# RedhawkSDR/psk_soft

Hardware: AMD Instinct MI355X
Metric: complex IQ Msamples/s, QPSK 8 sps, 4096 ch; % HBM roofline at 1/2/4/8 GPUs (higher is better)
Workload: dtype f32

## Files before the change

### psk_soft_amd/csrc/psk_capi.cpp

```cpp
#include <hip/hip_runtime_api.h>
#include <hip/hip_vector_types.h>

#include <atomic>
#include <cmath>
#include <condition_variable>
#include <cstdio>
#include <cstdlib>
#include <cstring>
#include <functional>
#include <mutex>
#include <new>
#include <string>
#include <thread>
#include <vector>

#include "psk_acquire.h"
#include "psk_symrate.h"
#include "psk_ctl.h"
#include "psk_gather.h"
#include "psk_plan.h"
#include "psk_quality.h"
#include "psk_soft_hip.h"
#include "psk_fir.h"
#include "psk_resample.h"
// ... 18 lines not shown
                             float2 *t_s, PfChan *pf_chan, uint32_t tile0, hipStream_t stream);
hipError_t launch_tile_front_any(const ChanPlan *plans, const uint32_t *list, uint32_t ch0, uint32_t nch, uint32_t max_tiles, uint32_t max_S,
                                 const ChanState *states, const float2 *rings, uint32_t ring_cap, TileInfo *tiles, float *t_raw, float2 *t_s,
                                 PfChan *pf_chan, hipStream_t stream);
hipError_t launch_tile_fit(const ChanPlan *plans, const uint32_t *list, uint32_t ch0, uint32_t nch, ChanState *states, float2 *rings,
                           uint32_t ring_cap, float *yvs, uint32_t fit_cap, uint32_t y_len, TileInfo *tiles, const float *t_raw,
                           const float2 *t_s, float *t_est, const PfScratch &sc, hipStream_t stream);
hipError_t launch_wide_front(const ChanPlan *plans, const uint32_t *list, uint32_t ch0, uint32_t nch, uint32_t max_tiles, uint32_t max_S,
                             const float2 *rings, uint32_t ring_cap, TileInfo *tiles, float *t_raw, float2 *t_s, PfChan *pf_chan, void *rec,
                             void *wst, hipStream_t stream);
size_t wide_rec_bytes();
size_t wide_stat_bytes();
uint32_t wide_chunks(uint32_t S);
hipError_t launch_seq_wide(const void *plans, const uint32_t *list, uint32_t ch0, uint32_t nch, void *states, float2 *rings,
                           uint32_t ring_cap, float *yvs, uint32_t fit_cap, double *symE, uint32_t symE_stride, hipStream_t stream);
hipError_t launch_pfit(const ChanPlan *plans, const uint32_t *list, uint32_t ch0, uint32_t nch, uint32_t max_tiles, ChanState *states,
                       float2 *rings, uint32_t ring_cap, float *yvs, uint32_t fit_cap, uint32_t y_len, TileInfo *tiles, const float *t_raw,
                       const float2 *t_s, float *t_est, const PfScratch &sc, bool second_round, hipStream_t stream);
hipError_t launch_tile_fit_range(const ChanPlan *plans, const uint32_t *list, uint32_t ch0, uint32_t nch, ChanState *states, float2 *rings,
                                 uint32_t ring_cap, float *yvs, uint32_t fit_cap, uint32_t y_len, TileInfo *tiles, const float *t_raw,
                                 const float2 *t_s, float *t_est, void *carry, float *carry_y, uint32_t tile0, uint32_t ntiles,
                                 hipStream_t stream);
size_t pipe_carry_bytes();
hipError_t launch_far_fit(const ChanPlan *plans, const uint32_t *list, uint32_t ch0, uint32_t nch, ChanState *states, float2 *rings,
                          uint32_t ring_cap, float *yvs, uint32_t fit_cap, float *far_y, uint32_t far_rows, TileInfo *tiles,
                          const float *t_raw, const float2 *t_s, float *t_est, hipStream_t stream);
hipError_t launch_far_quiet(const ChanPlan *plans, const uint32_t *list, uint32_t ch0, uint32_t nch, ChanState *states, float2 *rings,
                            uint32_t ring_cap, float *yvs, uint32_t fit_cap, float *far_y, uint32_t far_rows, hipStream_t stream);
size_t far_ring_bytes();
hipError_t launch_tile_back(const ChanPlan *plans, const uint32_t *list, uint32_t ch0, uint32_t nch, uint32_t max_tiles,
                            const ChanState *states, const TileInfo *tiles, const float2 *t_s, const float *t_est, uint32_t tile0,
                            uint32_t early, hipStream_t stream);
}
// ... 1024 lines not shown
    p.mode = p.S == 1u ? psk::PLAN_SEQ_S1 : psk::PLAN_SEQ;
    p.lf_flags &= ~(uint32_t)(psk::PLAN_TILED | psk::PLAN_PFIT | psk::PLAN_ANYFRONT | psk::PLAN_FARFIT);
}
psk_soft_status scratch_tiles(Round &r)
{
    psk_soft_handle *const h = r.h;
    PlanSummary &res = r.res;
    if (!r.tile_syms || (r.tile_syms <= h->tile_sym_cap && r.tile_count <= h->tile_cap && r.pf_syms <= h->pf_sym_cap && r.pf_count <= h->pf_cap))
        return PSK_SOFT_OK;
    h->tile_cap = h->tile_sym_cap = h->pf_cap = h->pf_sym_cap = 0;
    const size_t syms = plus_quarter(r.tile_syms), cnt = plus_quarter(r.tile_count);
    const size_t psyms = plus_quarter(r.pf_syms) + 128u, pcnt = plus_quarter(r.pf_count) + 1u;
    psk::PfScratch &pf = h->pf;
    bool got = false;
    PSK_HIP(grow_scratch({scratch_buf(&h->d_tiles, cnt), scratch_buf(&h->d_traw, syms), scratch_buf(&h->d_test, syms), scratch_buf(&h->d_ts, syms),
                          scratch_buf(&pf.k, psyms), scratch_buf(&pf.y, psyms), scratch_buf(&pf.S, psyms), scratch_buf(&pf.c, psyms),
                          scratch_buf(&pf.tt, psyms), scratch_buf(&pf.xs, psyms), scratch_buf(&pf.tile, pcnt),
                          scratch_buf(&pf.blk, psyms / 128u + 1u), scratch_buf(&pf.walk, psyms / 128u + 1u)},
                         &got));
    if (got && !pf.chan) {
        got = hipMalloc((void **)&pf.chan, sizeof(psk::PfChan) * h->nch) == hipSuccess &&
              hipMemset(pf.chan, 0, sizeof(psk::PfChan) * h->nch) == hipSuccess && hipHostMalloc((void **)&pf.hint, 64) == hipSuccess;
        if (got)
            *pf.hint = 0u;
    }
    if (got) {
        h->tile_cap = cnt, h->tile_sym_cap = syms, h->pf_cap = pcnt, h->pf_sym_cap = psyms;
        return PSK_SOFT_OK;
    }
    (void)hipGetLastError();
    for (uint32_t i = 0; i < r.nch; i++) {
        psk::ChanPlan &p = r.plans[i];
// ... 351 lines not shown
    psk_soft_handle *const h = r.h;
    const uint32_t *const l = r.d_list + s.off;
    const uint32_t ring_cap = h->lim.ring_cap, fit_cap = h->lim.fit_cap;
    PSK_HIP(mark(r, st, t.front, t.S, t.H, s.off, s.cnt, s.tiles_max, t.y_len, t.r_front));
    if (front == Front::window_class)
        PSK_HIP(psk::launch_tile_front(t.S, class_H(t.H), r.d_plans, l, r.ch0, s.cnt, s.tiles_max, h->d_state, h->d_ring, ring_cap, t.r_len, h->d_tiles,
                                       h->d_traw, h->d_ts, h->pf.chan, 0u, st));
    else if (front == Front::any)
        PSK_HIP(psk::launch_tile_front_any(r.d_plans, l, r.ch0, s.cnt, s.tiles_max, s.max_S, h->d_state, h->d_ring, ring_cap, h->d_tiles, h->d_traw,
                                           h->d_ts, h->pf.chan, st));
    else
        PSK_HIP(psk::launch_wide_front(r.d_plans, l, r.ch0, s.cnt, s.tiles_max, s.max_S, h->d_ring, ring_cap, h->d_tiles, h->d_traw, h->d_ts,
                                       h->pf.chan, h->d_wide_rec, h->d_wide_stat, st));
    if (fit == Fit::lds && h->opt_pfit) {
        PSK_HIP(mark(r, st, t.pfit, t.S, t.H, s.off, s.cnt, s.tiles_max, t.y_len, r.pf_second));
        PSK_HIP(psk::launch_pfit(r.d_plans, l, r.ch0, s.cnt, s.tiles_max, h->d_state, h->d_ring, ring_cap, h->d_yv, fit_cap, t.y_len, h->d_tiles,
                                 h->d_traw, h->d_ts, h->d_test, h->pf, r.pf_second, st));
    }
    PSK_HIP(mark(r, st, t.fit, t.S, t.H, s.off, s.cnt, s.tiles_max, t.y_len, t.r_len));
    if (fit == Fit::lds)
        PSK_HIP(psk::launch_tile_fit(r.d_plans, l, r.ch0, s.cnt, h->d_state, h->d_ring, ring_cap, h->d_yv, fit_cap, t.y_len, h->d_tiles, h->d_traw,
                                     h->d_ts, h->d_test, h->pf, st));
    else
        PSK_HIP(psk::launch_far_fit(r.d_plans, l, r.ch0, s.cnt, h->d_state, h->d_ring, ring_cap, h->d_yv, fit_cap, h->d_far_y, h->far_rows_cap,
                                    h->d_tiles, h->d_traw, h->d_ts, h->d_test, st));
    PSK_HIP(mark(r, st, t.back, t.S, t.H, s.off, s.cnt, s.tiles_max, t.y_len, t.r_len));
    PSK_HIP(psk::launch_tile_back(r.d_plans, l, r.ch0, s.cnt, s.tiles_max, h->d_state, h->d_tiles, h->d_ts, h->d_test, 0u, 0u, st));
    return PSK_SOFT_OK;
}
psk_soft_status enqueue_any_sets(const Round &r)
{
    psk_soft_handle *const h = r.h;
// ... 402 lines not shown
            if (h->ev_up[s]) (void)hipEventDestroy(h->ev_up[s]);
        }
        if (h->d_state) (void)hipFree(h->d_state);
        if (h->d_ring) (void)hipFree(h->d_ring);
        if (h->d_yv) (void)hipFree(h->d_yv);
        h->qpass.free();
        if (h->d_quality) (void)hipFree(h->d_quality);
        h->apass.free();
        if (h->d_acquire) (void)hipFree(h->d_acquire);
        h->spass.free();
        if (h->d_symrate) (void)hipFree(h->d_symrate);
        if (h->d_tiles) (void)hipFree(h->d_tiles);
        if (h->d_traw) (void)hipFree(h->d_traw);
        if (h->d_test) (void)hipFree(h->d_test);
        if (h->d_ts) (void)hipFree(h->d_ts);
        for (void *q : {(void *)h->pf.k, (void *)h->pf.y, (void *)h->pf.S, (void *)h->pf.c, (void *)h->pf.tt, (void *)h->pf.xs,
                        (void *)h->pf.tile, (void *)h->pf.blk, (void *)h->pf.walk, (void *)h->pf.chan})
            if (q) (void)hipFree(q);
        if (h->pf.hint) (void)hipHostFree(h->pf.hint);
        if (h->tile_ev) (void)hipEventDestroy(h->tile_ev);
        for (auto &cv : h->cvt) cv.free();
        for (auto &g : h->gat) g.free();
        for (auto &g : h->gdesc) g.free();
        if (h->d_tune_tab) (void)hipFree(h->d_tune_tab);
        h->rs_hist.free();
        if (h->d_fir_taps) (void)hipFree(h->d_fir_taps);
        h->fir_hist.free();
        for (auto &sl : h->stage) {
            if (sl.stream) (void)hipStreamSynchronize(sl.stream);
            if (sl.h_buf) (void)hipHostFree(sl.h_buf);
            if (sl.d_buf) (void)hipFree(sl.d_buf);
// ... 1959 lines not shown
```

### psk_soft_amd/csrc/psk_pfit.h

```cpp
#ifndef PSK_PFIT_H
#define PSK_PFIT_H

#include "psk_fast_kernel.h"

namespace psk {

constexpr uint32_t kPfFailYSum = 1u, kPfFailXySum = 2u, kPfFailUnwrap = 4u;

PSK_DEV bool pf_mine(const ChanPlan &p) { return p.mode == PLAN_FAST && (p.lf_flags & PLAN_PFIT) && p.n_out != 0; }
PSK_DEV bool pf_in_round(const ChanPlan &p, const PfScratch &sc, uint32_t bi, int round) { return pf_mine(p) && (round == 0 || sc.chan[bi].retry != 0u); }

struct PfGeo {
    int lane, n_out, n_blocks, c_begin, c_end, tile;
    uint64_t off;
    uint32_t tbase;
    uint32_t bbase;
};
PSK_DEV bool pf_geo(const ChanPlan &p, PfGeo &g)
{
    g.lane = threadIdx.x & 63;
    g.n_out = (int)p.n_out;
    g.n_blocks = (g.n_out + kB - 1) / kB;
    g.tile = (int)blockIdx.x;
    g.c_begin = g.tile * (int)p.tile_blocks;
    g.c_end = g.c_begin + (int)p.tile_blocks < g.n_blocks ? g.c_begin + (int)p.tile_blocks : g.n_blocks;
// ... 6 lines not shown
{
    const int n = (int)p.lf_n;
    return t >= n ? y_row[t - n] : yv[(p.lf_head + (uint32_t)t) % fit_cap];
}

constexpr float kPfSteep = 0.12f;
__global__ __launch_bounds__(64) void pf_unwrap_kernel(const ChanPlan *__restrict__ plans, const uint32_t *__restrict__ list, uint32_t ch0,
                                                       const ChanState *__restrict__ states, const float *__restrict__ t_raw, PfScratch sc)
{
    const uint32_t bi = list[blockIdx.y];
    const ChanPlan &p = plans[bi];
    PfGeo g;
    if (!pf_mine(p) || !pf_geo(p, g))
        return;
    const float *raw_row = t_raw + g.off;
    int *k_row = sc.k + g.off;
    const float inv2pi = 0.15915494f, two_pi = 6.2831853f;
    const ChanState &st = states[ch0 + bi];
    const bool steep = !(__builtin_fabsf(st.lf_m) < kPfSteep);
    int run = 0;
    if (steep) {
        for (int c = g.c_begin; c < g.c_end; c++) {
            const int i0 = c * kB + 2 * g.lane;
            const float2 rw = *reinterpret_cast<const float2 *>(raw_row + i0);
            const float before = c ? raw_row[c * kB - 1] : rw.x;
            const float prev = wave_up1(rw.y, before);
            int j0 = (int)__builtin_rintf((prev - rw.x) * inv2pi);
            const int j1 = (int)__builtin_rintf((rw.x - rw.y) * inv2pi);
            if (i0 == 0)
                j0 = 0;
            const int incl = wave_scan_i32(j0 + j1);
// ... 28 lines not shown
            const float U = a + two_pi * (float)(K - run);
            const float U_l = bperm_addr(((g.lane & ~7) - 8) << 2, U), U_r = bperm_addr(((g.lane & ~7) + 8) << 2, U);
            const float slope = grp == 0 ? (U_r - U) * (1.0f / 16.0f) : grp == 7 ? (U - U_l) * (1.0f / 16.0f) : (U_r - U_l) * (1.0f / 32.0f);
            const float dt0 = (float)(2 * (g.lane & 7)) - 7.5f;
            const float line0 = a + slope * dt0, line1 = line0 + slope;
            const int k0 = K + (int)__builtin_rintf((line0 - rw.x) * inv2pi), k1 = K + (int)__builtin_rintf((line1 - rw.y) * inv2pi);
            *reinterpret_cast<int2 *>(k_row + i0) = make_int2(k0, k1);
            run = __builtin_amdgcn_readlane(K, 63);
            a_last = read_lane(a, 63);
        }
    }
    if (g.lane == 0)
        sc.tile[g.tbase + g.tile].jsum = run;
}

__global__ __launch_bounds__(64) void pf_y_kernel(const ChanPlan *__restrict__ plans, const uint32_t *__restrict__ list, uint32_t ch0,
                                                  const ChanState *__restrict__ states, const float *__restrict__ t_raw, PfScratch sc, int round)
{
    const uint32_t bi = list[blockIdx.y];
    const ChanPlan &p = plans[bi];
    PfGeo g;
    if (!pf_in_round(p, sc, bi, round) || !pf_geo(p, g))
        return;
    const float *raw_row = t_raw + g.off;
    int *k_row = sc.k + g.off;
    float *y_row = sc.y + g.off;
    int koff = 0;
    if (round == 0) {
        for (int j = g.lane; j < g.tile; j += kWave) koff += sc.tile[g.tbase + j].jsum;
        koff = __builtin_amdgcn_readlane(wave_scan_i32(koff), 63);
        if (!(__builtin_fabsf(states[ch0 + bi].lf_m) < kPfSteep))
            koff += (int)unwrap_count(states[ch0 + bi].phaseEstimate, (double)raw_row[0]);
    }
    float2 rw_n = *reinterpret_cast<const float2 *>(raw_row + g.c_begin * kB + 2 * g.lane);
    int2 k_n = *reinterpret_cast<const int2 *>(k_row + g.c_begin * kB + 2 * g.lane);
    for (int c = g.c_begin; c < g.c_end; c++) {
        const int i0 = c * kB + 2 * g.lane;
        const float2 rw = rw_n;
        int2 k = k_n;
        if (c + 1 < g.c_end) {
            rw_n = *reinterpret_cast<const float2 *>(raw_row + i0 + kB);
            k_n = *reinterpret_cast<const int2 *>(k_row + i0 + kB);
        }
        k.x += koff;
        k.y += koff;
        *reinterpret_cast<int2 *>(k_row + i0) = k;
        const double two_pi = PSK_KD(kTwoPi, c);
        const float y0 = (float)((double)rw.x + (double)(long long)k.x * two_pi);
        const float y1 = (float)((double)rw.y + (double)(long long)k.y * two_pi);
        *reinterpret_cast<float2 *>(y_row + i0) = make_float2(y0, y1);
    }
}

__global__ __launch_bounds__(64) void pf_ydiff_kernel(const ChanPlan *__restrict__ plans, const uint32_t *__restrict__ list, uint32_t ch0,
                                                      const float *__restrict__ yvs, uint32_t fit_cap, PfScratch sc, int round)
{
    const uint32_t bi = list[blockIdx.y];
    const ChanPlan &p = plans[bi];
    PfGeo g;
    if (!pf_in_round(p, sc, bi, round) || !pf_geo(p, g))
        return;
    const float *y_row = sc.y + g.off;
    const float *yv = yvs + (size_t)(ch0 + bi) * fit_cap;
    double *S_row = sc.S + g.off;
    double run = 0.0, dlast = 0.0;
    const int j0 = g.c_begin * kB + 2 * g.lane;
    float2 y_n = *reinterpret_cast<const float2 *>(y_row + j0);
    float z0_n = pf_z(p, y_row, yv, fit_cap, j0), z1_n = pf_z(p, y_row, yv, fit_cap, j0 + 1);
    for (int c = g.c_begin; c < g.c_end; c++) {
        const int i0 = c * kB + 2 * g.lane;
        const float2 y = y_n;
        const float z0 = z0_n, z1 = z1_n;
        if (c + 1 < g.c_end) {
            y_n = *reinterpret_cast<const float2 *>(y_row + i0 + kB);
            z0_n = pf_z(p, y_row, yv, fit_cap, i0 + kB);
// ... 11 lines not shown
        dlast = read_lane((last & 1) ? a0 + d1 : a0, last >> 1);
    }
    if (g.lane == 0) {
        sc.tile[g.tbase + g.tile].dsum = run;
        sc.tile[g.tbase + g.tile].dlast = dlast;
    }
}

__global__ __launch_bounds__(64) void pf_ysum_kernel(const ChanPlan *__restrict__ plans, const uint32_t *__restrict__ list, uint32_t ch0,
                                                     const ChanState *__restrict__ states, const float *__restrict__ yvs, uint32_t fit_cap,
                                                     PfScratch sc, int round)
{
    const uint32_t bi = list[blockIdx.y];
    const ChanPlan &p = plans[bi];
    PfGeo g;
    if (!pf_in_round(p, sc, bi, round) || !pf_geo(p, g))
        return;
    const float *y_row = sc.y + g.off;
    const float *yv = yvs + (size_t)(ch0 + bi) * fit_cap;
    double *S_row = sc.S + g.off;
    double *c_row = sc.c + g.off;
    float *t_row = sc.tt + g.off;
    double soff = 0.0;
    for (int j = g.lane; j < g.tile; j += kWave) soff += sc.tile[g.tbase + j].dsum;
    soff = sc.chan[bi].ySum_c + wave_sum_f64(soff);
    bool bad = false;
    if (g.tile > 0) {
        double soff_b = 0.0;
        for (int j = g.lane; j < g.tile - 1; j += kWave) soff_b += sc.tile[g.tbase + j].dsum;
        soff_b = sc.chan[bi].ySum_c + wave_sum_f64(soff_b);
        bad = !same_bits(soff_b + sc.tile[g.tbase + g.tile - 1].dlast, soff);
    }
    const float xd = p.lf_xdelta;
    const float sizef = (float)(p.lf_n - 1u);
    double S_before = soff;
    double xrun = 0.0;
    const int j0 = g.c_begin * kB + 2 * g.lane;
// ... 11 lines not shown
            dl_n = *reinterpret_cast<const double2 *>(S_row + i0 + kB);
            z0_n = pf_z(p, y_row, yv, fit_cap, i0 + kB);
            z1_n = pf_z(p, y_row, yv, fit_cap, i0 + kB + 1);
        }
        const double S0 = soff + dl.x, S1 = soff + dl.y;
        const double z0 = v0 ? (double)z0f : 0.0, z1 = v1 ? (double)z1f : 0.0;
        const double Sp = wave_up1(S1, S_before);
        const double a0 = Sp - z0, a1 = S0 - z1;
        bad = bad || (v0 && !same_bits(a0 + (double)y.x, S0)) || (v1 && !same_bits(a1 + (double)y.y, S1));
        const double c0 = (double)xd * a0, c1 = (double)xd * a1;
        float t0 = y.x * sizef;
        t0 = t0 * xd;
        float t1 = y.y * sizef;
        t1 = t1 * xd;
        *reinterpret_cast<double2 *>(S_row + i0) = make_double2(S0, S1);
        *reinterpret_cast<double2 *>(c_row + i0) = make_double2(c0, c1);
        *reinterpret_cast<float2 *>(t_row + i0) = make_float2(t0, t1);
        const double bs = wave_sum_f64((v0 ? (double)t0 - c0 : 0.0) + (v1 ? (double)t1 - c1 : 0.0));
        if (g.lane == 0)
            sc.blk[g.bbase + c].bsum = bs;
        xrun += bs;
        const int rem = g.n_out - c * kB;
        const int last = (rem < kB ? rem : kB) - 1;
        S_before = read_lane((last & 1) ? S1 : S0, last >> 1);
    }
    if (g.lane == 0)
        sc.tile[g.tbase + g.tile].xsum = xrun;
    if (vote_any(bad) && g.lane == 0)
        atomicOr(&sc.chan[bi].fail, kPfFailYSum);
}

struct PfGrid {
// ... 33 lines not shown
    const unsigned long long lt = lane ? (~0ull >> (64 - lane)) : 0ull;
    const unsigned long long X = mA & lt, Y = mF & lt;
    const bool P_in = (X ? (Y > (X >> 1)) : P_c) != G;
    const bool sel0 = P_in != gr.E[0];
    const bool P0 = gr.T[0] ? gr.V[0] : (P_in != gr.V[0]);
    const bool sel1 = P0 != gr.E[1];
    if (!modeB) {
        a0 = gr.inc[0] + ((gr.T[0] && sel0) ? (gr.dpos[0] ? -1.0 : 1.0) : 0.0);
        a1 = gr.inc[1] + ((gr.T[1] && sel1) ? (gr.dpos[1] ? -1.0 : 1.0) : 0.0);
    } else {
        a0 = gr.inc[0] + (gr.T[0] ? (sel0 ? 1.0 : -1.0) : 0.0);
        a1 = gr.inc[1] + (gr.T[1] ? (sel1 ? 1.0 : -1.0) : 0.0);
    }
}

__global__ __launch_bounds__(64) void pf_xblock_kernel(const ChanPlan *__restrict__ plans, const uint32_t *__restrict__ list, uint32_t ch0,
                                                       const ChanState *__restrict__ states, PfScratch sc, int round)
{
    const uint32_t bi = list[blockIdx.y];
    const ChanPlan &p = plans[bi];
    PfGeo g;
    if (!pf_in_round(p, sc, bi, round) || !pf_geo(p, g))
        return;
    const double *c_row = sc.c + g.off;
    const float *t_row = sc.tt + g.off;
    double s_pred = 0.0;
    for (int j = g.lane; j < g.tile; j += kWave) s_pred += sc.tile[g.tbase + j].xsum;
    s_pred = sc.chan[bi].xySum_c + wave_sum_f64(s_pred);
    int prev_scale = -1;
    if (g.c_begin > 0) {
        const double s_before = s_pred - sc.blk[g.bbase + g.c_begin - 1].bsum;
        const int eb_b = (__double2hiint(s_before - c_row[(g.c_begin - 1) * kB]) >> 20) & 0x7ff;
        if (eb_b >= 60 && eb_b <= 2040)
            prev_scale = 2 * eb_b + (!(__builtin_fabs(s_before) < pow2_biased(eb_b + 1)) ? 1 : 0);
    }
    for (int c = g.c_begin; c < g.c_end; c++) {
        const int i0 = c * kB + 2 * g.lane;
        const bool v0 = i0 < g.n_out, v1 = i0 + 1 < g.n_out;
        const double2 cv = *reinterpret_cast<const double2 *>(c_row + i0);
        const float2 tv = *reinterpret_cast<const float2 *>(t_row + i0);
        const double cc[kR] = {v0 ? cv.x : 0.0, v1 ? cv.y : 0.0};
        const double tt[kR] = {v0 ? (double)tv.x : 0.0, v1 ? (double)tv.y : 0.0};
        const double c_first = read_lane(cc[0], 0);
        const double r_first = s_pred - c_first;
        const int eb = (__double2hiint(r_first) >> 20) & 0x7ff;
        PfBlock rec;
        rec.bsum = sc.blk[g.bbase + c].bsum;
        rec.a = __builtin_inf();
        rec.b = -__builtin_inf();
        rec.kmul = rec.D0s = rec.D1s = 0.0;
        rec.flags = rec.pad = 0;
        int scale_id = -1;
        if (eb >= 60 && eb <= 2040) {
            const double inv_q = pow2_biased(2098 - eb);
            const bool modeB = !(__builtin_fabs(s_pred) < pow2_biased(eb + 1));
// ... 45 lines not shown
        }
        prev_scale = scale_id;
        if (g.lane == 0)
            sc.blk[g.bbase + c] = rec;
        s_pred += rec.bsum;
    }
}

PSK_DEV bool pf_x_ok(double s_c, const bool (&valid)[kR], const double (&c)[kR], const double (&t)[kR], const double (&xs)[kR])
{
    const double xp = wave_up1(xs[1], s_c);
    const bool x0 = same_bits((xp - c[0]) + t[0], xs[0]), x1 = same_bits((xs[0] - c[1]) + t[1], xs[1]);
    return vote_all((x0 || !valid[0]) && (x1 || !valid[1]));
}

struct PfOps {
    double2 cv;
    float2 tv;
};
PSK_DEV PfOps pf_load_ops(int lane, int b, const double *c_row, const float *t_row)
{
    const int i0 = b * kB + 2 * lane;
    PfOps o;
    o.cv = *reinterpret_cast<const double2 *>(c_row + i0);
    o.tv = *reinterpret_cast<const float2 *>(t_row + i0);
    return o;
}
PSK_DEV double pf_walk_block(int lane, int b, int n_out, double s_c, const PfOps &ops, double *xs_row, bool try_grid, bool &grid_failed)
{
    const int i0 = b * kB + 2 * lane;
    const bool valid[kR] = {i0 < n_out, i0 + 1 < n_out};
#ifdef PSK_DIAG_WALK_NOLOAD
    const double2 cv = make_double2(s_c * 0.25, s_c * 0.125);
    const float2 tv = make_float2((float)lane, 1.0f);
#else
    const double2 cv = ops.cv;
    const float2 tv = ops.tv;
#endif
    const double cc[kR] = {valid[0] ? cv.x : 0.0, valid[1] ? cv.y : 0.0};
    const double tt[kR] = {valid[0] ? (double)tv.x : 0.0, valid[1] ? (double)tv.y : 0.0};
    double xs[kR];
    bool done = false;
// ... 19 lines not shown
        const double b_fin = wave_up1(x, s_c);
        xs[0] = (b_fin - cc[0]) + tt[0];
        xs[1] = x;
    }
    *reinterpret_cast<double2 *>(xs_row + i0) = make_double2(xs[0], xs[1]);
    const int rem = n_out - b * kB;
    const int last = (rem < kB ? rem : kB) - 1;
    return read_lane((last & 1) ? xs[1] : xs[0], last >> 1);
}

PSK_DEV double pf_from_lane(double v, int src)
{
    const int lo = bperm_addr(src << 2, __double2loint(v)), hi = bperm_addr(src << 2, __double2hiint(v));
    return __hiloint2double(hi, lo);
}
__global__ __launch_bounds__(64) void pf_xwalk_kernel(const ChanPlan *__restrict__ plans, const uint32_t *__restrict__ list,
                                                      const PfBlock *__restrict__ blk_all, PfScratch sc, int round)
{
    const uint32_t bi = list[blockIdx.x];
    const ChanPlan &p = plans[bi];
    if (!pf_in_round(p, sc, bi, round))
        return;
    const int lane = threadIdx.x & 63;
    const int n_out = (int)p.n_out;
    const int n_blocks = (n_out + kB - 1) / kB;
    const PfBlock *const blk = blk_all + (uint32_t)(p.tile_off / kB);
    PfWalk *const walk = sc.walk + (uint32_t)(p.tile_off / kB);
    const double *c_row = sc.c + p.tile_off;
    const float *t_row = sc.tt + p.tile_off;
    double *xs_row = sc.xs + p.tile_off;
    double s_c = sc.chan[bi].xySum_c;
    uint32_t slow_blocks = 0;
#ifdef PSK_DIAG_WALK_TIME
    const unsigned long long t_begin = wall_clock64();
#endif
    int par = -1;
    for (int b0 = 0; b0 < n_blocks; b0 += kWave) {
        const bool have = b0 + lane < n_blocks;
        const PfBlock rec = blk[have ? b0 + lane : n_blocks - 1];
        const int nb = n_blocks - b0 < kWave ? n_blocks - b0 : kWave;
        const bool usable = have && rec.a < rec.b;
        double s_in_mine = 0.0;
        int slow_mine = 0;
        int start = 0;
// ... 33 lines not shown
            if (lane >= start && lane < f)
                s_in_mine = s_before;
            if (f > start) {
                s_c = read_lane(s_after, f - 1);
                par = __builtin_amdgcn_readlane(par_after, f - 1);
            }
            if (f >= nb)
                break;
            const double a_f = read_lane(rec.a, f), b_f = read_lane(rec.b, f);
            if (a_f < s_c && s_c < b_f && f > start) {
                par = -1;
                start = f;
                continue;
            }
            int fs = f;
            PfOps ops = pf_load_ops(lane, b0 + fs, c_row, t_row);
            bool grid_first = !(a_f < b_f);
            bool grid_failed = false;
            for (;;) {
                const bool more = fs + 1 < nb;
                PfOps ahead = ops;
                if (more)
                    ahead = pf_load_ops(lane, b0 + fs + 1, c_row, t_row);
                if (lane == fs) {
                    s_in_mine = s_c;
                    slow_mine = 1;
                }
                s_c = pf_walk_block(lane, b0 + fs, n_out, s_c, ops, xs_row, grid_first, grid_failed);
                slow_blocks++;
                start = fs + 1;
                if (!more)
                    break;
                const double a_n = read_lane(rec.a, fs + 1), b_n = read_lane(rec.b, fs + 1);
                if (a_n < s_c && s_c < b_n)
                    break;
                fs++;
                ops = ahead;
                grid_first = !(a_n < b_n) && !grid_failed;
            }
            par = -1;
        }
        if (have) {
            PfWalk w;
// ... 107 lines not shown
```

### psk_soft_amd/csrc/psk_plan.h

```cpp
#ifndef PSK_PLAN_H
#define PSK_PLAN_H

#include <stdint.h>

#define PSK_PKT_ID_cs16 1
#define PSK_PKT_ID_cs8 3
#define PSK_PKT_ID_cf16 4

namespace psk {

enum PlanMode : uint32_t {
    PLAN_SKIP = 0,
    PLAN_FAST = 1,
    PLAN_SEQ = 2,
    PLAN_SEQ_S1 = 3,
};

enum LfFlags : uint32_t {
    LF_RECOMPUTE = 1u,
    PLAN_QPSK_SIGN_MAP = 2u,
    PLAN_TILED = 4u,
    PLAN_PFIT = 8u,
    PLAN_ANYFRONT = 16u,
    PLAN_NO_WRAP = 32u,
// ... 86 lines not shown
    double D0s, D1s;
    int flags;
    int pad;
};
struct PfWalk {
    double s_in;
    int slow;
    int pad;
};
struct PfChan {
    uint32_t fail, done, slow_blocks;
    uint32_t retry;
    double ySum_c, xySum_c;
};
struct PfScratch {
    int *k;
    float *y;
    double *S;
    double *c;
    float *tt;
    double *xs;
    PfTile *tile;
    PfBlock *blk;
    PfWalk *walk;
    PfChan *chan;
    uint32_t *hint;
};

struct ChanState {
    double lf_ySum;
    double lf_xySum;
    float last_re;
    float last_im;
    float phaseEstimate;
    float lf_den;
// ... 17 lines not shown
```

### psk_soft_amd/csrc/psk_tile.hip

```cpp
#include "psk_tile_kernel.h"
#include "psk_pfit.h"
#include "psk_tile_any.h"

namespace psk {

constexpr int kAnyPhases = 16;
template <int NP>
__global__ __launch_bounds__(64) void psk_tile_front_any_kernel(const ChanPlan *__restrict__ plans, const uint32_t *__restrict__ list, uint32_t ch0,
                                                                const ChanState *__restrict__ states, const float2 *__restrict__ rings,
                                                                uint32_t ring_cap, TileInfo *__restrict__ tiles, float *__restrict__ t_raw,
                                                                float2 *__restrict__ t_s, PfChan *__restrict__ pf_chan)
{
    const int lane = threadIdx.x & 63;
    const uint32_t bi = list[blockIdx.y];
    const ChanPlan &p = plans[bi];
    if (!tile_plan_mine(p) || !(p.lf_flags & PLAN_ANYFRONT))
        return;
    const int n_out = (int)p.n_out;
    const int n_blocks = (n_out + kB - 1) / kB;
    const int c_begin = (int)(blockIdx.x * p.tile_blocks);
    if (c_begin >= n_blocks)
        return;
    if (blockIdx.x == 0 && lane == 0)
        pf_chan[bi].fail = pf_chan[bi].done = pf_chan[bi].slow_blocks = pf_chan[bi].retry = 0u;
// ... 666 lines not shown

hipError_t launch_tile_fit(const ChanPlan *plans, const uint32_t *list, uint32_t ch0, uint32_t nch, ChanState *states, float2 *rings,
                           uint32_t ring_cap, float *yvs, uint32_t fit_cap, uint32_t y_len, TileInfo *tiles, const float *t_raw,
                           const float2 *t_s, float *t_est, const PfScratch &sc, hipStream_t stream)
{
    if (!nch)
        return hipSuccess;
    static LdsGrant granted;
    if (const hipError_t e = lds_grant(reinterpret_cast<const void *>(&psk_tile_fit_kernel), sizeof(float) * (size_t)y_len, granted))
        return e;
    hipLaunchKernelGGL(psk_tile_fit_kernel, dim3(nch), dim3(kWave), sizeof(float) * (size_t)y_len, stream, plans, list, ch0, states, rings,
                       ring_cap, yvs, fit_cap, y_len, tiles, t_raw, t_s, t_est, sc);
    return hipGetLastError();
}

hipError_t launch_pfit(const ChanPlan *plans, const uint32_t *list, uint32_t ch0, uint32_t nch, uint32_t max_tiles, ChanState *states,
                       float2 *rings, uint32_t ring_cap, float *yvs, uint32_t fit_cap, uint32_t y_len, TileInfo *tiles, const float *t_raw,
                       const float2 *t_s, float *t_est, const PfScratch &sc, bool second_round, hipStream_t stream)
{
    if (!nch || !max_tiles)
        return hipSuccess;
    const dim3 wave(kWave);
    static LdsGrant granted_b;
    if (const hipError_t e = lds_grant(reinterpret_cast<const void *>(&pf_begin_kernel), sizeof(float) * (size_t)y_len, granted_b))
        return e;
    for (uint32_t off = 0; off < nch; off += kGridYMax) {
        const uint32_t n = nch - off < kGridYMax ? nch - off : kGridYMax;
        const uint32_t *const l = list + off;
        const dim3 grid(max_tiles, n);
        hipLaunchKernelGGL(pf_begin_kernel, dim3(n), wave, sizeof(float) * (size_t)y_len, stream, plans, l, ch0, states, yvs, fit_cap, y_len, sc);
        hipLaunchKernelGGL(pf_unwrap_kernel, grid, wave, 0, stream, plans, l, ch0, states, t_raw, sc);
        for (int round = 0; round <= (second_round ? 1 : 0); round++) {
            if (round)
                hipLaunchKernelGGL(pf_retry_kernel, dim3(n), wave, 0, stream, plans, l, sc);
            hipLaunchKernelGGL(pf_y_kernel, grid, wave, 0, stream, plans, l, ch0, states, t_raw, sc, round);
            hipLaunchKernelGGL(pf_ydiff_kernel, grid, wave, 0, stream, plans, l, ch0, yvs, fit_cap, sc, round);
            hipLaunchKernelGGL(pf_ysum_kernel, grid, wave, 0, stream, plans, l, ch0, states, yvs, fit_cap, sc, round);
            hipLaunchKernelGGL(pf_xblock_kernel, grid, wave, 0, stream, plans, l, ch0, states, sc, round);
            hipLaunchKernelGGL(pf_xwalk_kernel, dim3(n), wave, 0, stream, plans, l, sc.blk, sc, round);
            hipLaunchKernelGGL(pf_verify_kernel, grid, wave, 0, stream, plans, l, ch0, states, yvs, fit_cap, t_raw, t_est, sc, round);
        }
    }
    return hipGetLastError();
}

hipError_t launch_tile_back(const ChanPlan *plans, const uint32_t *list, uint32_t ch0, uint32_t nch, uint32_t max_tiles,
                            const ChanState *states, const TileInfo *tiles, const float2 *t_s, const float *t_est, uint32_t tile0,
                            uint32_t early, hipStream_t stream)
{
    if (!nch || !max_tiles)
        return hipSuccess;
    for (uint32_t off = 0; off < nch; off += kGridYMax) {
        const uint32_t n = nch - off < kGridYMax ? nch - off : kGridYMax;
        hipLaunchKernelGGL(psk_tile_back_kernel, dim3(max_tiles, n), dim3(kWave), 0, stream, plans, list + off, ch0, states, tiles, t_s, t_est, tile0, early);
// ... 6 lines not shown
```

Before: 472,300.

## Fuse pfit y/ydiff/ysum kernels into one LDS-halo sums kernel and recompute ops

Adds pf_sums_kernel, which unwraps phase, builds y, computes the running sums and per-block x-sums in a single launch per tile. It stages a halo of prior samples in LDS so each tile can rebuild its prefix offset without a separate diff pass. It also drops the c and tt scratch arrays, recomputing those operands from S and y inside xblock and xwalk. The goal is fewer launches and less scratch traffic. The cost is redundant halo reads, extra recomputation, a new cross-tile consistency check, and the old path kept for large tiles or windows.

```diff
diff --git a/psk_soft_amd/csrc/psk_capi.cpp b/psk_soft_amd/csrc/psk_capi.cpp
--- a/psk_soft_amd/csrc/psk_capi.cpp
+++ b/psk_soft_amd/csrc/psk_capi.cpp
@@ -56,9 +56,10 @@
 uint32_t wide_chunks(uint32_t S);
 hipError_t launch_seq_wide(const void *plans, const uint32_t *list, uint32_t ch0, uint32_t nch, void *states, float2 *rings,
                            uint32_t ring_cap, float *yvs, uint32_t fit_cap, double *symE, uint32_t symE_stride, hipStream_t stream);
-hipError_t launch_pfit(const ChanPlan *plans, const uint32_t *list, uint32_t ch0, uint32_t nch, uint32_t max_tiles, ChanState *states,
-                       float2 *rings, uint32_t ring_cap, float *yvs, uint32_t fit_cap, uint32_t y_len, TileInfo *tiles, const float *t_raw,
-                       const float2 *t_s, float *t_est, const PfScratch &sc, bool second_round, hipStream_t stream);
+hipError_t launch_pfit(const ChanPlan *plans, const uint32_t *list, uint32_t ch0, uint32_t nch, uint32_t max_tiles, uint32_t tile_blocks,
+                       uint32_t max_n, ChanState *states, float2 *rings, uint32_t ring_cap, float *yvs, uint32_t fit_cap, uint32_t y_len,
+                       TileInfo *tiles, const float *t_raw, const float2 *t_s, float *t_est, const PfScratch &sc, bool second_round,
+                       hipStream_t stream);
 hipError_t launch_tile_fit_range(const ChanPlan *plans, const uint32_t *list, uint32_t ch0, uint32_t nch, ChanState *states, float2 *rings,
                                  uint32_t ring_cap, float *yvs, uint32_t fit_cap, uint32_t y_len, TileInfo *tiles, const float *t_raw,
                                  const float2 *t_s, float *t_est, void *carry, float *carry_y, uint32_t tile0, uint32_t ntiles,
@@ -1113,8 +1114,8 @@
     psk::PfScratch &pf = h->pf;
     bool got = false;
     PSK_HIP(grow_scratch({scratch_buf(&h->d_tiles, cnt), scratch_buf(&h->d_traw, syms), scratch_buf(&h->d_test, syms), scratch_buf(&h->d_ts, syms),
-                          scratch_buf(&pf.k, psyms), scratch_buf(&pf.y, psyms), scratch_buf(&pf.S, psyms), scratch_buf(&pf.c, psyms),
-                          scratch_buf(&pf.tt, psyms), scratch_buf(&pf.xs, psyms), scratch_buf(&pf.tile, pcnt),
+                          scratch_buf(&pf.kr, psyms), scratch_buf(&pf.k, psyms), scratch_buf(&pf.y, psyms), scratch_buf(&pf.S, psyms),
+                          scratch_buf(&pf.xs, psyms), scratch_buf(&pf.tile, pcnt),
                           scratch_buf(&pf.blk, psyms / 128u + 1u), scratch_buf(&pf.walk, psyms / 128u + 1u)},
                          &got));
     if (got && !pf.chan) {
@@ -1496,8 +1497,8 @@
                                        h->pf.chan, h->d_wide_rec, h->d_wide_stat, st));
     if (fit == Fit::lds && h->opt_pfit) {
         PSK_HIP(mark(r, st, t.pfit, t.S, t.H, s.off, s.cnt, s.tiles_max, t.y_len, r.pf_second));
-        PSK_HIP(psk::launch_pfit(r.d_plans, l, r.ch0, s.cnt, s.tiles_max, h->d_state, h->d_ring, ring_cap, h->d_yv, fit_cap, t.y_len, h->d_tiles,
-                                 h->d_traw, h->d_ts, h->d_test, h->pf, r.pf_second, st));
+        PSK_HIP(psk::launch_pfit(r.d_plans, l, r.ch0, s.cnt, s.tiles_max, s.K, s.max_n, h->d_state, h->d_ring, ring_cap, h->d_yv, fit_cap, t.y_len,
+                                 h->d_tiles, h->d_traw, h->d_ts, h->d_test, h->pf, r.pf_second, st));
     }
     PSK_HIP(mark(r, st, t.fit, t.S, t.H, s.off, s.cnt, s.tiles_max, t.y_len, t.r_len));
     if (fit == Fit::lds)
@@ -1930,7 +1931,7 @@
         if (h->d_traw) (void)hipFree(h->d_traw);
         if (h->d_test) (void)hipFree(h->d_test);
         if (h->d_ts) (void)hipFree(h->d_ts);
-        for (void *q : {(void *)h->pf.k, (void *)h->pf.y, (void *)h->pf.S, (void *)h->pf.c, (void *)h->pf.tt, (void *)h->pf.xs,
+        for (void *q : {(void *)h->pf.kr, (void *)h->pf.k, (void *)h->pf.y, (void *)h->pf.S, (void *)h->pf.xs,
                         (void *)h->pf.tile, (void *)h->pf.blk, (void *)h->pf.walk, (void *)h->pf.chan})
             if (q) (void)hipFree(q);
         if (h->pf.hint) (void)hipHostFree(h->pf.hint);
diff --git a/psk_soft_amd/csrc/psk_pfit.h b/psk_soft_amd/csrc/psk_pfit.h
--- a/psk_soft_amd/csrc/psk_pfit.h
+++ b/psk_soft_amd/csrc/psk_pfit.h
@@ -9,6 +9,8 @@
 
 PSK_DEV bool pf_mine(const ChanPlan &p) { return p.mode == PLAN_FAST && (p.lf_flags & PLAN_PFIT) && p.n_out != 0; }
 PSK_DEV bool pf_in_round(const ChanPlan &p, const PfScratch &sc, uint32_t bi, int round) { return pf_mine(p) && (round == 0 || sc.chan[bi].retry != 0u); }
+constexpr uint32_t kPfFusedBlocks = 16u;
+PSK_DEV bool pf_fused(const ChanPlan &p) { return p.tile_blocks <= kPfFusedBlocks && p.lf_n <= p.tile_blocks * (uint32_t)kB; }
 
 struct PfGeo {
     int lane, n_out, n_blocks, c_begin, c_end, tile;
@@ -45,7 +47,7 @@
     if (!pf_mine(p) || !pf_geo(p, g))
         return;
     const float *raw_row = t_raw + g.off;
-    int *k_row = sc.k + g.off;
+    int *k_row = sc.kr + g.off;
     const float inv2pi = 0.15915494f, two_pi = 6.2831853f;
     const ChanState &st = states[ch0 + bi];
     const bool steep = !(__builtin_fabsf(st.lf_m) < kPfSteep);
@@ -104,15 +106,134 @@
         sc.tile[g.tbase + g.tile].jsum = run;
 }
 
-__global__ __launch_bounds__(64) void pf_y_kernel(const ChanPlan *__restrict__ plans, const uint32_t *__restrict__ list, uint32_t ch0,
-                                                  const ChanState *__restrict__ states, const float *__restrict__ t_raw, PfScratch sc, int round)
-{
+__global__ __launch_bounds__(64) void pf_sums_kernel(const ChanPlan *__restrict__ plans, const uint32_t *__restrict__ list, uint32_t ch0,
+                                                     const ChanState *__restrict__ states, const float *__restrict__ t_raw,
+                                                     const float *__restrict__ yvs, uint32_t fit_cap, uint32_t halo, PfScratch sc, int round)
+{
+    extern __shared__ __attribute__((aligned(16))) float pf_lds[];
     const uint32_t bi = list[blockIdx.y];
     const ChanPlan &p = plans[bi];
     PfGeo g;
-    if (!pf_in_round(p, sc, bi, round) || !pf_geo(p, g))
-        return;
+    if (!pf_in_round(p, sc, bi, round) || !pf_fused(p) || !pf_geo(p, g))
+        return;
+    const int n = (int)p.lf_n;
+    if (n > (int)halo) {
+        if (g.lane == 0)
+            atomicOr(&sc.chan[bi].fail, kPfFailYSum);
+        return;
+    }
     const float *raw_row = t_raw + g.off;
+    const int *k_in = (round == 0 ? sc.kr : sc.k) + g.off;
+    int *k_row = sc.k + g.off;
+    float *y_row = sc.y + g.off;
+    double *S_row = sc.S + g.off;
+    const int t0 = g.c_begin * kB;
+    float *const yt = pf_lds + halo;
+    int koff = 0, koff_prev = 0;
+    if (round == 0) {
+        for (int j = g.lane; j < g.tile - 1; j += kWave) koff_prev += sc.tile[g.tbase + j].jsum;
+        koff_prev = __builtin_amdgcn_readlane(wave_scan_i32(koff_prev), 63);
+        if (!(__builtin_fabsf(states[ch0 + bi].lf_m) < kPfSteep))
+            koff_prev += (int)unwrap_count(states[ch0 + bi].phaseEstimate, (double)raw_row[0]);
+        koff = koff_prev + (g.tile > 0 ? sc.tile[g.tbase + g.tile - 1].jsum : 0);
+    }
+    {
+        const float *yv = yvs + (size_t)(ch0 + bi) * fit_cap;
+        const double two_pi = PSK_KD(kTwoPi, t0);
+        for (int m = 1 + g.lane; m <= n; m += kWave) {
+            float v;
+            if (g.tile == 0) {
+                v = yv[(p.lf_head + (uint32_t)(n - m)) % fit_cap];
+            } else {
+                const int t = t0 - m;
+                v = (float)((double)raw_row[t] + (double)(long long)(k_in[t] + koff_prev) * two_pi);
+            }
+            yt[-m] = v;
+        }
+    }
+    {
+        float2 rw_n = *reinterpret_cast<const float2 *>(raw_row + t0 + 2 * g.lane);
+        int2 k_n = *reinterpret_cast<const int2 *>(k_in + t0 + 2 * g.lane);
+        for (int c = g.c_begin; c < g.c_end; c++) {
+            const int i0 = c * kB + 2 * g.lane;
+            const float2 rw = rw_n;
+            int2 k = k_n;
+            if (c + 1 < g.c_end) {
+                rw_n = *reinterpret_cast<const float2 *>(raw_row + i0 + kB);
+                k_n = *reinterpret_cast<const int2 *>(k_in + i0 + kB);
+            }
+            k.x += koff;
+            k.y += koff;
+            if (round == 0)
+                *reinterpret_cast<int2 *>(k_row + i0) = k;
+            const double two_pi = PSK_KD(kTwoPi, c);
+            const float y0 = (float)((double)rw.x + (double)(long long)k.x * two_pi);
+            const float y1 = (float)((double)rw.y + (double)(long long)k.y * two_pi);
+            *reinterpret_cast<float2 *>(y_row + i0) = make_float2(y0, y1);
+            *reinterpret_cast<float2 *>(yt + (i0 - t0)) = make_float2(y0, y1);
+        }
+    }
+    __syncthreads();
+    double soff;
+    if (g.tile == 0) {
+        soff = sc.chan[bi].ySum_c + 0.0;
+    } else {
+        double w = 0.0;
+        for (int m = 1 + g.lane; m <= n; m += kWave) w += (double)yt[-m];
+        soff = wave_sum_f64(w);
+    }
+    const float xd = p.lf_xdelta;
+    const float sizef = (float)(p.lf_n - 1u);
+    bool bad = false;
+    double run = 0.0;
+    double S_before = soff;
+    double xrun = 0.0;
+    for (int c = g.c_begin; c < g.c_end; c++) {
+        const int i0 = c * kB + 2 * g.lane;
+        const int li = i0 - t0;
+        const bool v0 = i0 < g.n_out, v1 = i0 + 1 < g.n_out;
+        const float2 y = *reinterpret_cast<const float2 *>(yt + li);
+        const float z0f = yt[li - n], z1f = yt[li + 1 - n];
+        const double d0 = v0 ? (double)y.x - (double)z0f : 0.0;
+        const double d1 = v1 ? (double)y.y - (double)z1f : 0.0;
+        const double incl = wave_scan_f64(d0 + d1);
+        const double p0 = (run + wave_up1(incl, 0.0)) + d0, p1 = p0 + d1;
+        run += read_lane(incl, 63);
+        const double S0 = soff + p0, S1 = soff + p1;
+        const double z0 = v0 ? (double)z0f : 0.0, z1 = v1 ? (double)z1f : 0.0;
+        const double Sp = wave_up1(S1, S_before);
+        const double a0 = Sp - z0, a1 = S0 - z1;
+        bad = bad || (v0 && !same_bits(a0 + (double)y.x, S0)) || (v1 && !same_bits(a1 + (double)y.y, S1));
+        const double c0 = (double)xd * a0, c1 = (double)xd * a1;
+        float t0f = y.x * sizef;
+        t0f = t0f * xd;
+        float t1f = y.y * sizef;
+        t1f = t1f * xd;
+        *reinterpret_cast<double2 *>(S_row + i0) = make_double2(S0, S1);
+        const double bs = wave_sum_f64((v0 ? (double)t0f - c0 : 0.0) + (v1 ? (double)t1f - c1 : 0.0));
+        if (g.lane == 0)
+            sc.blk[g.bbase + c].bsum = bs;
+        xrun += bs;
+        const int rem = g.n_out - c * kB;
+        const int last = (rem < kB ? rem : kB) - 1;
+        S_before = read_lane((last & 1) ? S1 : S0, last >> 1);
+    }
+    if (g.lane == 0)
+        sc.tile[g.tbase + g.tile].xsum = xrun;
+    if (vote_any(bad) && g.lane == 0)
+        atomicOr(&sc.chan[bi].fail, kPfFailYSum);
+}
+
+__global__ __launch_bounds__(64) void pf_y_kernel(const ChanPlan *__restrict__ plans, const uint32_t *__restrict__ list, uint32_t ch0,
+                                                  const ChanState *__restrict__ states, const float *__restrict__ t_raw, PfScratch sc, int round)
+{
+    const uint32_t bi = list[blockIdx.y];
+    const ChanPlan &p = plans[bi];
+    PfGeo g;
+    if (!pf_in_round(p, sc, bi, round) || pf_fused(p) || !pf_geo(p, g))
+        return;
+    const float *raw_row = t_raw + g.off;
+    const int *k_in = (round == 0 ? sc.kr : sc.k) + g.off;
     int *k_row = sc.k + g.off;
     float *y_row = sc.y + g.off;
     int koff = 0;
@@ -123,14 +244,14 @@
             koff += (int)unwrap_count(states[ch0 + bi].phaseEstimate, (double)raw_row[0]);
     }
     float2 rw_n = *reinterpret_cast<const float2 *>(raw_row + g.c_begin * kB + 2 * g.lane);
-    int2 k_n = *reinterpret_cast<const int2 *>(k_row + g.c_begin * kB + 2 * g.lane);
+    int2 k_n = *reinterpret_cast<const int2 *>(k_in + g.c_begin * kB + 2 * g.lane);
     for (int c = g.c_begin; c < g.c_end; c++) {
         const int i0 = c * kB + 2 * g.lane;
         const float2 rw = rw_n;
         int2 k = k_n;
         if (c + 1 < g.c_end) {
             rw_n = *reinterpret_cast<const float2 *>(raw_row + i0 + kB);
-            k_n = *reinterpret_cast<const int2 *>(k_row + i0 + kB);
+            k_n = *reinterpret_cast<const int2 *>(k_in + i0 + kB);
         }
         k.x += koff;
         k.y += koff;
@@ -148,7 +269,7 @@
     const uint32_t bi = list[blockIdx.y];
     const ChanPlan &p = plans[bi];
     PfGeo g;
-    if (!pf_in_round(p, sc, bi, round) || !pf_geo(p, g))
+    if (!pf_in_round(p, sc, bi, round) || pf_fused(p) || !pf_geo(p, g))
         return;
     const float *y_row = sc.y + g.off;
     const float *yv = yvs + (size_t)(ch0 + bi) * fit_cap;
@@ -190,13 +311,11 @@
     const uint32_t bi = list[blockIdx.y];
     const ChanPlan &p = plans[bi];
     PfGeo g;
-    if (!pf_in_round(p, sc, bi, round) || !pf_geo(p, g))
+    if (!pf_in_round(p, sc, bi, round) || pf_fused(p) || !pf_geo(p, g))
         return;
     const float *y_row = sc.y + g.off;
     const float *yv = yvs + (size_t)(ch0 + bi) * fit_cap;
     double *S_row = sc.S + g.off;
-    double *c_row = sc.c + g.off;
-    float *t_row = sc.tt + g.off;
     double soff = 0.0;
     for (int j = g.lane; j < g.tile; j += kWave) soff += sc.tile[g.tbase + j].dsum;
     soff = sc.chan[bi].ySum_c + wave_sum_f64(soff);
@@ -238,8 +357,6 @@
         float t1 = y.y * sizef;
         t1 = t1 * xd;
         *reinterpret_cast<double2 *>(S_row + i0) = make_double2(S0, S1);
-        *reinterpret_cast<double2 *>(c_row + i0) = make_double2(c0, c1);
-        *reinterpret_cast<float2 *>(t_row + i0) = make_float2(t0, t1);
         const double bs = wave_sum_f64((v0 ? (double)t0 - c0 : 0.0) + (v1 ? (double)t1 - c1 : 0.0));
         if (g.lane == 0)
             sc.blk[g.bbase + c].bsum = bs;
@@ -303,31 +420,80 @@
     }
 }
 
+struct PfOps {
+    double2 cv;
+    float2 tv;
+};
+struct PfOpsIn {
+    double2 Sv;
+    float2 y;
+    double S_front;
+    float z0, z1;
+};
+PSK_DEV PfOpsIn pf_load_ops_in(const ChanPlan &p, int lane, int b, double ySum_c, const double *S_row, const float *y_row, const float *yv, uint32_t fit_cap)
+{
+    const int i0 = b * kB + 2 * lane;
+    PfOpsIn in;
+    in.Sv = *reinterpret_cast<const double2 *>(S_row + i0);
+    in.y = *reinterpret_cast<const float2 *>(y_row + i0);
+    in.S_front = b ? S_row[b * kB - 1] : ySum_c + 0.0;
+    in.z0 = pf_z(p, y_row, yv, fit_cap, i0);
+    in.z1 = pf_z(p, y_row, yv, fit_cap, i0 + 1);
+    return in;
+}
+PSK_DEV PfOps pf_form_ops(const ChanPlan &p, const PfOpsIn &in)
+{
+    const double Sp = wave_up1(in.Sv.y, in.S_front);
+    const double a0 = Sp - (double)in.z0, a1 = in.Sv.x - (double)in.z1;
+    const float xd = p.lf_xdelta;
+    const float sizef = (float)(p.lf_n - 1u);
+    float t0 = in.y.x * sizef;
+    t0 = t0 * xd;
+    float t1 = in.y.y * sizef;
+    t1 = t1 * xd;
+    PfOps o;
+    o.cv = make_double2((double)xd * a0, (double)xd * a1);
+    o.tv = make_float2(t0, t1);
+    return o;
+}
+
 __global__ __launch_bounds__(64) void pf_xblock_kernel(const ChanPlan *__restrict__ plans, const uint32_t *__restrict__ list, uint32_t ch0,
-                                                       const ChanState *__restrict__ states, PfScratch sc, int round)
+                                                       const ChanState *__restrict__ states, const float *__restrict__ yvs, uint32_t fit_cap,
+                                                       PfScratch sc, int round)
 {
     const uint32_t bi = list[blockIdx.y];
     const ChanPlan &p = plans[bi];
     PfGeo g;
     if (!pf_in_round(p, sc, bi, round) || !pf_geo(p, g))
         return;
-    const double *c_row = sc.c + g.off;
-    const float *t_row = sc.tt + g.off;
+    const double *S_row = sc.S + g.off;
+    const float *y_row = sc.y + g.off;
+    const float *yv = yvs + (size_t)(ch0 + bi) * fit_cap;
+    const double ySum_c = sc.chan[bi].ySum_c;
+    if (pf_fused(p) && g.tile > 0) {
+        const int t = g.c_begin * kB;
+        const double z = (double)pf_z(p, y_row, yv, fit_cap, t);
+        if (!same_bits((S_row[t - 1] - z) + (double)y_row[t], S_row[t]) && g.lane == 0)
+            atomicOr(&sc.chan[bi].fail, kPfFailYSum);
+    }
     double s_pred = 0.0;
     for (int j = g.lane; j < g.tile; j += kWave) s_pred += sc.tile[g.tbase + j].xsum;
     s_pred = sc.chan[bi].xySum_c + wave_sum_f64(s_pred);
     int prev_scale = -1;
     if (g.c_begin > 0) {
         const double s_before = s_pred - sc.blk[g.bbase + g.c_begin - 1].bsum;
-        const int eb_b = (__double2hiint(s_before - c_row[(g.c_begin - 1) * kB]) >> 20) & 0x7ff;
+        const int tb = (g.c_begin - 1) * kB;
+        const double c_b = (double)p.lf_xdelta * ((tb ? S_row[tb - 1] : ySum_c + 0.0) - (double)pf_z(p, y_row, yv, fit_cap, tb));
+        const int eb_b = (__double2hiint(s_before - c_b) >> 20) & 0x7ff;
         if (eb_b >= 60 && eb_b <= 2040)
             prev_scale = 2 * eb_b + (!(__builtin_fabs(s_before) < pow2_biased(eb_b + 1)) ? 1 : 0);
     }
     for (int c = g.c_begin; c < g.c_end; c++) {
         const int i0 = c * kB + 2 * g.lane;
         const bool v0 = i0 < g.n_out, v1 = i0 + 1 < g.n_out;
-        const double2 cv = *reinterpret_cast<const double2 *>(c_row + i0);
-        const float2 tv = *reinterpret_cast<const float2 *>(t_row + i0);
+        const PfOps ops = pf_form_ops(p, pf_load_ops_in(p, g.lane, c, ySum_c, S_row, y_row, yv, fit_cap));
+        const double2 cv = ops.cv;
+        const float2 tv = ops.tv;
         const double cc[kR] = {v0 ? cv.x : 0.0, v1 ? cv.y : 0.0};
         const double tt[kR] = {v0 ? (double)tv.x : 0.0, v1 ? (double)tv.y : 0.0};
         const double c_first = read_lane(cc[0], 0);
@@ -403,18 +569,6 @@
     return vote_all((x0 || !valid[0]) && (x1 || !valid[1]));
 }
 
-struct PfOps {
-    double2 cv;
-    float2 tv;
-};
-PSK_DEV PfOps pf_load_ops(int lane, int b, const double *c_row, const float *t_row)
-{
-    const int i0 = b * kB + 2 * lane;
-    PfOps o;
-    o.cv = *reinterpret_cast<const double2 *>(c_row + i0);
-    o.tv = *reinterpret_cast<const float2 *>(t_row + i0);
-    return o;
-}
 PSK_DEV double pf_walk_block(int lane, int b, int n_out, double s_c, const PfOps &ops, double *xs_row, bool try_grid, bool &grid_failed)
 {
     const int i0 = b * kB + 2 * lane;
@@ -464,7 +618,8 @@
     const int lo = bperm_addr(src << 2, __double2loint(v)), hi = bperm_addr(src << 2, __double2hiint(v));
     return __hiloint2double(hi, lo);
 }
-__global__ __launch_bounds__(64) void pf_xwalk_kernel(const ChanPlan *__restrict__ plans, const uint32_t *__restrict__ list,
+__global__ __launch_bounds__(64) void pf_xwalk_kernel(const ChanPlan *__restrict__ plans, const uint32_t *__restrict__ list, uint32_t ch0,
+                                                      const float *__restrict__ yvs, uint32_t fit_cap,
                                                       const PfBlock *__restrict__ blk_all, PfScratch sc, int round)
 {
     const uint32_t bi = list[blockIdx.x];
@@ -476,8 +631,10 @@
     const int n_blocks = (n_out + kB - 1) / kB;
     const PfBlock *const blk = blk_all + (uint32_t)(p.tile_off / kB);
     PfWalk *const walk = sc.walk + (uint32_t)(p.tile_off / kB);
-    const double *c_row = sc.c + p.tile_off;
-    const float *t_row = sc.tt + p.tile_off;
+    const double *S_row = sc.S + p.tile_off;
+    const float *y_row = sc.y + p.tile_off;
+    const float *yv = yvs + (size_t)(ch0 + bi) * fit_cap;
+    const double ySum_c = sc.chan[bi].ySum_c;
     double *xs_row = sc.xs + p.tile_off;
     double s_c = sc.chan[bi].xySum_c;
     uint32_t slow_blocks = 0;
@@ -541,19 +698,19 @@
                 continue;
             }
             int fs = f;
-            PfOps ops = pf_load_ops(lane, b0 + fs, c_row, t_row);
+            PfOpsIn ops = pf_load_ops_in(p, lane, b0 + fs, ySum_c, S_row, y_row, yv, fit_cap);
             bool grid_first = !(a_f < b_f);
             bool grid_failed = false;
             for (;;) {
                 const bool more = fs + 1 < nb;
-                PfOps ahead = ops;
+                PfOpsIn ahead = ops;
                 if (more)
-                    ahead = pf_load_ops(lane, b0 + fs + 1, c_row, t_row);
+                    ahead = pf_load_ops_in(p, lane, b0 + fs + 1, ySum_c, S_row, y_row, yv, fit_cap);
                 if (lane == fs) {
                     s_in_mine = s_c;
                     slow_mine = 1;
                 }
-                s_c = pf_walk_block(lane, b0 + fs, n_out, s_c, ops, xs_row, grid_first, grid_failed);
+                s_c = pf_walk_block(lane, b0 + fs, n_out, s_c, pf_form_ops(p, ops), xs_row, grid_first, grid_failed);
                 slow_blocks++;
                 start = fs + 1;
                 if (!more)
diff --git a/psk_soft_amd/csrc/psk_plan.h b/psk_soft_amd/csrc/psk_plan.h
--- a/psk_soft_amd/csrc/psk_plan.h
+++ b/psk_soft_amd/csrc/psk_plan.h
@@ -124,11 +124,10 @@
     double ySum_c, xySum_c;
 };
 struct PfScratch {
+    int *kr;
     int *k;
     float *y;
     double *S;
-    double *c;
-    float *tt;
     double *xs;
     PfTile *tile;
     PfBlock *blk;
diff --git a/psk_soft_amd/csrc/psk_tile.hip b/psk_soft_amd/csrc/psk_tile.hip
--- a/psk_soft_amd/csrc/psk_tile.hip
+++ b/psk_soft_amd/csrc/psk_tile.hip
@@ -704,9 +704,10 @@
     return hipGetLastError();
 }
 
-hipError_t launch_pfit(const ChanPlan *plans, const uint32_t *list, uint32_t ch0, uint32_t nch, uint32_t max_tiles, ChanState *states,
-                       float2 *rings, uint32_t ring_cap, float *yvs, uint32_t fit_cap, uint32_t y_len, TileInfo *tiles, const float *t_raw,
-                       const float2 *t_s, float *t_est, const PfScratch &sc, bool second_round, hipStream_t stream)
+hipError_t launch_pfit(const ChanPlan *plans, const uint32_t *list, uint32_t ch0, uint32_t nch, uint32_t max_tiles, uint32_t tile_blocks,
+                       uint32_t max_n, ChanState *states, float2 *rings, uint32_t ring_cap, float *yvs, uint32_t fit_cap, uint32_t y_len,
+                       TileInfo *tiles, const float *t_raw, const float2 *t_s, float *t_est, const PfScratch &sc, bool second_round,
+                       hipStream_t stream)
 {
     if (!nch || !max_tiles)
         return hipSuccess;
@@ -714,6 +715,10 @@
     static LdsGrant granted_b;
     if (const hipError_t e = lds_grant(reinterpret_cast<const void *>(&pf_begin_kernel), sizeof(float) * (size_t)y_len, granted_b))
         return e;
+    const uint32_t tile_syms = tile_blocks * (uint32_t)kB;
+    const bool some_fused = tile_blocks <= kPfFusedBlocks, all_fused = some_fused && max_n <= tile_syms;
+    const uint32_t halo = ((max_n < tile_syms ? max_n : tile_syms) + 3u) & ~3u;
+    const size_t sums_lds = sizeof(float) * (size_t)(halo + tile_syms);
     for (uint32_t off = 0; off < nch; off += kGridYMax) {
         const uint32_t n = nch - off < kGridYMax ? nch - off : kGridYMax;
         const uint32_t *const l = list + off;
@@ -723,11 +728,15 @@
         for (int round = 0; round <= (second_round ? 1 : 0); round++) {
             if (round)
                 hipLaunchKernelGGL(pf_retry_kernel, dim3(n), wave, 0, stream, plans, l, sc);
-            hipLaunchKernelGGL(pf_y_kernel, grid, wave, 0, stream, plans, l, ch0, states, t_raw, sc, round);
-            hipLaunchKernelGGL(pf_ydiff_kernel, grid, wave, 0, stream, plans, l, ch0, yvs, fit_cap, sc, round);
-            hipLaunchKernelGGL(pf_ysum_kernel, grid, wave, 0, stream, plans, l, ch0, states, yvs, fit_cap, sc, round);
-            hipLaunchKernelGGL(pf_xblock_kernel, grid, wave, 0, stream, plans, l, ch0, states, sc, round);
-            hipLaunchKernelGGL(pf_xwalk_kernel, dim3(n), wave, 0, stream, plans, l, sc.blk, sc, round);
+            if (some_fused)
+                hipLaunchKernelGGL(pf_sums_kernel, grid, wave, sums_lds, stream, plans, l, ch0, states, t_raw, yvs, fit_cap, halo, sc, round);
+            if (!all_fused) {
+                hipLaunchKernelGGL(pf_y_kernel, grid, wave, 0, stream, plans, l, ch0, states, t_raw, sc, round);
+                hipLaunchKernelGGL(pf_ydiff_kernel, grid, wave, 0, stream, plans, l, ch0, yvs, fit_cap, sc, round);
+                hipLaunchKernelGGL(pf_ysum_kernel, grid, wave, 0, stream, plans, l, ch0, states, yvs, fit_cap, sc, round);
+            }
+            hipLaunchKernelGGL(pf_xblock_kernel, grid, wave, 0, stream, plans, l, ch0, states, yvs, fit_cap, sc, round);
+            hipLaunchKernelGGL(pf_xwalk_kernel, dim3(n), wave, 0, stream, plans, l, ch0, yvs, fit_cap, sc.blk, sc, round);
             hipLaunchKernelGGL(pf_verify_kernel, grid, wave, 0, stream, plans, l, ch0, states, yvs, fit_cap, t_raw, t_est, sc, round);
         }
     }
```

New measurement: 449,300. -4.9%, worse.
